# webmproject/sjpeg

Hardware: AMD Instinct MI355X
Metric: Mpixels/s JPEG encode, 4K RGB q=75 YUV420; bit-exact vs ref (higher is better)
Workload: dtype int32/int16 (u8 in); 1 GPU; 64 device-resident 3840x2160 G_struct frames per GPU per step, q=75 YUV420 method 0 (standard Huffman), one complete JPEG per frame; frames_per_gpu=64, width=3840, height=2160, yuv_mode=420, parallelism=frame-sharded x1, no data-path collective, pipelined=True

## Files before the change

sjpeg_amd/csrc/stitch_kernels.h:

```cpp

struct StitchArgs {
  int nseg, nframes;
  const uint32_t* seg_nbits;
  unsigned long long* seg_off;
  const uint32_t* seg_words;
  uint32_t slot_words;
  const uint32_t* pool;
  uint32_t pool_words;
  const uint32_t* seg_xbase;
  const uint32_t* pool_ctr;
  uint32_t* ubuf;
  size_t ubuf_words;
  uint32_t* chunk_ff;
  unsigned long long* chunk_off;
  uint32_t max_chunks;
  const uint8_t* header;
  uint32_t header_size;
  const uint32_t* hdr_off;
  int append_eoi;
  uint8_t* out;
  size_t out_stride;
  unsigned long long* sizes;
  unsigned long long* pack_off = nullptr;
  const unsigned long long* seg_nbits64;
  unsigned long long* total_bits_out;
  uint32_t subs;
  uint32_t wide_subs;
  int seg_first;
  int rst_tail;
  uint32_t* frame_flags;
  int fused_k4;
  int fused_k2;
  const RaggedFrame* rframes = nullptr;
  const uint32_t* rmap_place = nullptr;
  const uint32_t* rmap_stuff = nullptr;
};

__device__ __forceinline__ StitchArgs ragged_stitch_view(const StitchArgs& in, uint32_t f) {
  const RaggedFrame& d = in.rframes[f];
  StitchArgs v = in;
  v.nseg = d.nseg; v.nframes = 1;
  v.seg_nbits = in.seg_nbits + d.seg_base;
  v.seg_off = in.seg_off + d.seg_base + f;
  v.seg_words = in.seg_words + static_cast<size_t>(d.seg_base) * in.slot_words;
  v.pool = in.pool + d.pool_base; v.pool_words = d.pool_words;
  v.seg_xbase = in.seg_xbase + d.seg_base;
  v.pool_ctr = in.pool_ctr + 2 * f;
  v.ubuf = in.ubuf + d.ubuf_base; v.ubuf_words = d.ubuf_words;
  v.chunk_ff = in.chunk_ff + d.chunk_base; v.chunk_off = in.chunk_off + d.chunk_base; v.max_chunks = d.max_chunks;
  if (in.hdr_off != nullptr) v.hdr_off = in.hdr_off + f;
  v.out = in.out + d.out_offset; v.out_stride = d.out_capacity;
  v.sizes = in.sizes + f;
  v.frame_flags = in.frame_flags + f;
  return v;
}
__device__ __forceinline__ bool frame_overran(const StitchArgs& a, int frame) {
  if (a.pool_ctr == nullptr) return false;
  return a.frame_flags != nullptr ? a.frame_flags[frame] != 0u : a.pool_ctr[2 * frame + 1] != 0u;
}

template <bool RAGGED = false>
__global__ __launch_bounds__(kThreads) void scan_seg_offsets(const StitchArgs a_in) {
  __shared__ uint32_t scratch[16];
  const StitchArgs a = RAGGED ? ragged_stitch_view(a_in, blockIdx.x) : a_in;
  const int frame = RAGGED ? 0 : blockIdx.x;
  const uint32_t* nb = a.seg_nbits + static_cast<size_t>(frame) * a.nseg;
  unsigned long long* off = a.seg_off + static_cast<size_t>(frame) * (a.nseg + 1);
  auto len_of = [&](int i) -> uint32_t {
    return a.seg_nbits64 != nullptr ? static_cast<uint32_t>(a.seg_nbits64[static_cast<size_t>(frame) * a.nseg + i]) : nb[i];
  };
  constexpr int kRun = 8;
  unsigned long long running = 0;
  for (int base = 0; base < a.nseg; base += kThreads * kRun) {
    const int i0 = base + static_cast<int>(threadIdx.x) * kRun;
    uint32_t v[kRun];
    unsigned long long mine = 0;
#pragma unroll
    for (int j = 0; j < kRun; ++j) {
      v[j] = (i0 + j < a.nseg) ? len_of(i0 + j) : 0u;
      mine += v[j];
    }
    unsigned long long at, round_total;
    if (a.seg_nbits64 == nullptr) {
      uint32_t total;
      const uint32_t ex = wg_exclusive_scan<kThreads>(static_cast<uint32_t>(mine), scratch, &total);
      at = running + ex;
      round_total = total;
    } else {
      uint32_t total_lo, total_hi;
      const uint32_t ex_lo = wg_exclusive_scan<kThreads>(static_cast<uint32_t>(mine & 0xffffffu), scratch, &total_lo);
      const uint32_t ex_hi = wg_exclusive_scan<kThreads>(static_cast<uint32_t>(mine >> 24), scratch, &total_hi);
      at = running + ex_lo + (static_cast<unsigned long long>(ex_hi) << 24);
      round_total = total_lo + (static_cast<unsigned long long>(total_hi) << 24);
    }
#pragma unroll
    for (int j = 0; j < kRun; ++j) {
      if (i0 + j < a.nseg) off[i0 + j] = at;
      at += v[j];
    }
    running += round_total;
  }
  if (threadIdx.x == 0) {
    off[a.nseg] = running;
    if (a.total_bits_out != nullptr) a.total_bits_out[frame] = running;
  }
  const unsigned long long U = (running + 7) >> 3;
  unsigned long long nch64 = (U + kChunkBytes - 1) / kChunkBytes;
  if (nch64 > a.max_chunks) nch64 = a.max_chunks;
  const uint32_t nchunks = static_cast<uint32_t>(nch64);
  uint32_t* ff = a.chunk_ff + static_cast<size_t>(frame) * a.max_chunks;
  for (uint32_t i = threadIdx.x; i < nchunks; i += kThreads) ff[i] = 0;
  if (a.frame_flags != nullptr && a.pool_ctr != nullptr && threadIdx.x == 0) {
    a.frame_flags[frame] = a.pool_ctr[2 * frame + 1];
    const_cast<uint32_t*>(a.pool_ctr)[2 * frame] = 0u;
    const_cast<uint32_t*>(a.pool_ctr)[2 * frame + 1] = 0u;
  }
}


__device__ __forceinline__ uint32_t ff_bytes(uint32_t w) {
  return ((w & 0x7f7f7f7fu) + 0x01010101u) & w & 0x80808080u;
}
__device__ __forceinline__ uint32_t count_ff(uint32_t w, int nbytes ) {
  uint32_t n = 0;
#pragma unroll
  for (int b = 0; b < 4; ++b) {
    if (b < nbytes && ((w >> (24 - 8 * b)) & 0xffu) == 0xffu) ++n;
  }
  return n;
}

constexpr int kSpec = 12;
constexpr int kPlaceLanes = 64;
constexpr int kWideSpec = 3;
struct __attribute__((packed, aligned(4))) Words4 { uint32_t w[4]; };
constexpr int kFusedSegs = 2048;
constexpr int kFusedSegsBig = 16384;
template <int FUSED, bool RAGGED = false>
__global__ __launch_bounds__(kThreads) void place_segments(const StitchArgs a_in) {
  __shared__ uint32_t off_lds[FUSED == 1 ? kFusedSegs + 1 : 16];
  __shared__ uint32_t scratch_k2[16];
  const uint32_t rf = RAGGED ? a_in.rmap_place[blockIdx.x] : 0u;
  const uint32_t bx = RAGGED ? blockIdx.x - a_in.rframes[rf].place_base : blockIdx.x;
  const StitchArgs a = RAGGED ? ragged_stitch_view(a_in, rf) : a_in;
  const int frame = RAGGED ? 0 : blockIdx.y;
  const uint32_t* const nb_f = a.seg_nbits + static_cast<size_t>(frame) * a.nseg;
  const int sc_first = static_cast<int>((bx * (kThreads / 64)) / a.subs);
  if (FUSED == 1) {
    const uint32_t* const nb = nb_f;
    constexpr int kRun = kFusedSegs / kThreads;
    const int i0 = static_cast<int>(threadIdx.x) * kRun;
    uint32_t v[kRun], mine = 0;
#pragma unroll
    for (int j = 0; j < kRun; ++j) {
      v[j] = (i0 + j < a.nseg) ? nb[i0 + j] : 0u;
      mine += v[j];
    }
    uint32_t total;
    uint32_t at = wg_exclusive_scan<kThreads>(mine, scratch_k2, &total);
#pragma unroll
    for (int j = 0; j < kRun; ++j) { off_lds[i0 + j] = at; at += v[j]; }
    if (threadIdx.x == 0) {
      off_lds[a.nseg] = total;
      if (bx == 0) {
        a.seg_off[static_cast<size_t>(frame) * (a.nseg + 1) + a.nseg] = total;
        if (a.frame_flags != nullptr && a.pool_ctr != nullptr) a.frame_flags[frame] = a.pool_ctr[2 * frame + 1];
      }
    }
    __syncthreads();
  }
  if (FUSED == 2) {
    uint32_t front = 0, all = 0;
    for (int i = threadIdx.x; i < a.nseg; i += kThreads) {
      const uint32_t v = nb_f[i];
      all += v;
      front += i < sc_first ? v : 0u;
    }
    uint32_t front_total, all_total;
    (void)wg_exclusive_scan<kThreads>(front, scratch_k2, &front_total);
    (void)wg_exclusive_scan<kThreads>(all, scratch_k2, &all_total);
    if (threadIdx.x < 8) {
      uint32_t at = front_total;
      for (int j = 0; j < static_cast<int>(threadIdx.x); ++j) at += sc_first + j < a.nseg ? nb_f[sc_first + j] : 0u;
      off_lds[threadIdx.x] = at;
    }
    if (threadIdx.x == 8) {
      off_lds[8] = all_total;
      if (bx == 0) {
        a.seg_off[static_cast<size_t>(frame) * (a.nseg + 1) + a.nseg] = all_total;
        if (a.frame_flags != nullptr && a.pool_ctr != nullptr) a.frame_flags[frame] = a.pool_ctr[2 * frame + 1];
      }
    }
    __syncthreads();
  }
  const uint32_t unit = bx * (kThreads / kPlaceLanes) + (threadIdx.x >> 6);
  const int sc0 = static_cast<int>(unit / a.subs);
  const uint32_t ibase = (unit % a.subs) * (a.wide_subs ? kWideSpec * 256u : kSpec * kPlaceLanes);
  if (sc0 >= a.nseg) return;
  const unsigned long long* const off_g = a.seg_off + static_cast<size_t>(frame) * (a.nseg + 1);
  auto off = [&](int i) -> unsigned long long {
    if (FUSED == 1) return off_lds[i];
    if (FUSED == 2) {
      if (i >= a.nseg) return off_lds[8];
      if (i - sc_first < 8) return off_lds[i - sc_first];
      unsigned long long at = off_lds[7];
      for (int j = sc_first + 7; j < i; ++j) at += nb_f[j];
      return at;
    }
    return off_g[i];
  };
  const uint32_t* segw = a.seg_words + static_cast<size_t>(frame) * a.nseg * a.slot_words;
  const uint32_t* src = segw + static_cast<size_t>(sc0) * a.slot_words;
  const bool wide = (a.subs == 1u || a.wide_subs) && (a.slot_words & 3u) == 0u && a.slot_words >= 776u;
  uint32_t spec[kSpec][2];
  uint4 wq[kWideSpec];
  uint32_t wx[kWideSpec];
  if (wide) {
#pragma unroll
    for (int k = 0; k < kWideSpec; ++k) {
      const uint32_t i = min(ibase + 256u * k + 4u * (threadIdx.x & 63), a.slot_words - 4u);
      wq[k] = *reinterpret_cast<const uint4*>(src + i);
      wx[k] = src[min(i + 4u, a.slot_words - 1u)];
    }
  } else {
#pragma unroll
    for (int k = 0; k < kSpec; ++k) {
      const uint32_t i = min(ibase + k * kPlaceLanes + (threadIdx.x & 63), a.slot_words - 2u);
      spec[k][0] = src[i];
      spec[k][1] = src[i + 1];
    }
  }
  const bool has_next = sc0 + 1 < a.nseg;
  const uint32_t next_first = has_next ? src[a.slot_words] : 0u;
  const unsigned long long b0 = off(sc0), b1 = off(sc0 + 1);
  const unsigned long long b2 = off(has_next ? sc0 + 2 : sc0 + 1);
  const unsigned long long T = off(a.nseg);
  const unsigned long long U = (T + 7) >> 3;
  const bool overran = FUSED ? (a.pool_ctr != nullptr && a.pool_ctr[2 * frame + 1] != 0u) : frame_overran(a, frame);
  if (((U + 3) >> 2) + 1 > a.ubuf_words || overran) return;
  const uint32_t* const pool_f = a.pool == nullptr ? nullptr : a.pool + static_cast<size_t>(frame) * a.pool_words;
  const uint32_t* const xbase_f = a.seg_xbase == nullptr ? nullptr : a.seg_xbase + static_cast<size_t>(frame) * a.nseg;
  auto seg_word = [&](int sc, uint32_t i) -> uint32_t {
    if (i < a.slot_words) return segw[static_cast<size_t>(sc) * a.slot_words + i];
    if (xbase_f == nullptr) return 0u;
    const uint32_t xb = xbase_f[sc];
    return xb == 0xffffffffu ? 0u : pool_f[xb + (i - a.slot_words)];
  };
  uint32_t* ub = a.ubuf + static_cast<size_t>(frame) * a.ubuf_words;
  uint32_t* cff = a.chunk_ff + static_cast<size_t>(frame) * a.max_chunks;
  const int lane = threadIdx.x & 63;
  const unsigned long long wbeg = (b0 + 31) >> 5;
  const unsigned long long wend = (sc0 == a.nseg - 1) ? ((U + 3) >> 2) : ((b1 + 31) >> 5);
  const uint32_t nwords = static_cast<uint32_t>(wend - wbeg);
  const uint32_t lead = static_cast<uint32_t>(wbeg * 32 - b0);
  const uint32_t len = static_cast<uint32_t>(b1 - b0);
  uint32_t* dst = ub + wbeg;
  const uint32_t wbase = static_cast<uint32_t>(wbeg);
  uint32_t ff_acc = 0;
  uint32_t ff_chunk = 0xffffffffu;
  auto ff_flush = [&]() {
    uint32_t sum = ff_acc;
    for (int d = 32; d > 0; d >>= 1) sum += __shfl_down(sum, d, 64);
    if (lane == 0 && sum != 0u) atomicAdd(&cff[ff_chunk], sum);
    ff_acc = 0;
  };
  auto gather_word = [&](uint32_t i) -> uint32_t {
    uint32_t outw = 0;
    int need = 32, sc = sc0;
    unsigned long long p = (wbeg + i) * 32, c_beg = b0, c_end = b1;
    while (need > 0 && p < T) {
      while (p >= c_end) { ++sc; c_beg = c_end; c_end = off(sc + 1); }
      const unsigned long long avail = c_end - p;
      const int take = avail < static_cast<unsigned long long>(need) ? static_cast<int>(avail) : need;
      const uint32_t rr = static_cast<uint32_t>(p - c_beg);
      const unsigned long long two = (static_cast<unsigned long long>(seg_word(sc, rr >> 5)) << 32) | seg_word(sc, (rr >> 5) + 1);
      const uint32_t bits = static_cast<uint32_t>((two << (rr & 31)) >> (64 - take));
      outw |= bits << (need - take);
      need -= take;
      p += take;
    }
    if (need > 0) outw |= (need == 32) ? 0xffffffffu : ((1u << need) - 1u);
    return outw;
  };
  auto one = [&](uint32_t i, uint32_t v0, uint32_t v1) {
    uint32_t ffs = 0;
    if (i < nwords) {
      const uint32_t r = lead + 32u * i;
      uint32_t outw;
      if (r + 32u <= len) {
        outw = lead ? __builtin_amdgcn_alignbit(v0, v1, 32u - lead) : v0;
      } else {
        outw = gather_word(i);
      }
      dst[i] = outw;
      const unsigned long long byte0 = (wbeg + i) * 4;
      const int valid = byte0 >= U ? 0 : (U - byte0 >= 4 ? 4 : static_cast<int>(U - byte0));
      ffs = valid == 4 ? static_cast<uint32_t>(__popc(ff_bytes(outw))) : count_ff(outw, valid);
    }
    const uint32_t chunk = (wbase + i) >> 10;
    const uint32_t chunk0 = __builtin_amdgcn_readfirstlane(chunk);
    if (chunk0 != ff_chunk) {
      if (ff_chunk != 0xffffffffu) ff_flush();
      ff_chunk = chunk0;
    }
    if (chunk == chunk0) ff_acc += ffs;
    else if (ffs != 0u) atomicAdd(&cff[chunk], ffs);
  };
  const bool long_seg = ((len + lead + 31u) >> 5) + 2u > a.slot_words;
  if (!long_seg && wide) {
    const uint32_t n_int = len >= lead + 32u ? (len - lead) >> 5 : 0u;
    const uint32_t edge_bits = len > lead ? (len - lead) & 31u : 0u;
    const bool edge_easy = !has_next || (b2 - b1) >= 32u - edge_bits;
    const unsigned long long edge_byte0 = (wbeg + n_int) * 4;
    const uint32_t edge_valid = edge_byte0 >= U ? 0u : (U - edge_byte0 >= 4 ? 4u : static_cast<uint32_t>(U - edge_byte0));
    auto batch = [&](uint32_t i0, uint4 q, uint32_t x) {
      const uint32_t i = i0 + 4u * lane;
      const uint32_t v[5] = {q.x, q.y, q.z, q.w, x};
      const bool full = i0 + 256u <= n_int;
      Words4 o;
      uint32_t f[4];
#pragma unroll
      for (int u = 0; u < 4; ++u) {
        o.w[u] = lead ? __builtin_amdgcn_alignbit(v[u], v[u + 1], 32u - lead) : v[u];
        f[u] = static_cast<uint32_t>(__popc(ff_bytes(o.w[u])));
      }
      if (full) {
        *reinterpret_cast<Words4*>(dst + i) = o;
      } else {
        const bool edge_here = n_int < nwords && n_int >= i0 && n_int < i0 + 256u;
        const uint32_t gathered = (edge_here && !edge_easy) ? gather_word(n_int) : 0u;
        const uint32_t hi_mask = edge_bits ? ~(0xffffffffu >> edge_bits) : 0u;
        const uint32_t tail = (has_next ? next_first : 0xffffffffu) >> edge_bits;
#pragma unroll
        for (int u = 0; u < 4; ++u) {
          const uint32_t idx = i + u;
          if (edge_here && idx == n_int) {
            o.w[u] = edge_easy ? ((o.w[u] & hi_mask) | tail) : gathered;
            f[u] = edge_valid == 4u ? static_cast<uint32_t>(__popc(ff_bytes(o.w[u]))) : count_ff(o.w[u], static_cast<int>(edge_valid));
          }
          if (idx < nwords) dst[idx] = o.w[u]; else f[u] = 0;
        }
      }
      const uint32_t ffs = f[0] + f[1] + f[2] + f[3];
      const uint32_t c_lo = (wbase + i) >> 10, c_hi = (wbase + i + 3u) >> 10;
      const uint32_t chunk0 = __builtin_amdgcn_readfirstlane(c_lo);
      if (chunk0 != ff_chunk) {
        if (ff_chunk != 0xffffffffu) ff_flush();
        ff_chunk = chunk0;
      }
      if (c_lo == chunk0 && c_hi == chunk0) {
        ff_acc += ffs;
      } else if (ffs != 0u) {
#pragma unroll
        for (int u = 0; u < 4; ++u) {
          const uint32_t c = (wbase + i + u) >> 10;
          if (f[u] != 0u) { if (c == chunk0) ff_acc += f[u]; else atomicAdd(&cff[c], f[u]); }
        }
      }
    };
#pragma unroll
    for (int k = 0; k < kWideSpec; ++k) {
      if (ibase + 256u * k < nwords) batch(ibase + 256u * k, wq[k], wx[k]);
    }
    if (a.wide_subs) { if (ff_chunk != 0xffffffffu) ff_flush(); return; }
    auto fetch = [&](uint32_t i0, uint4* q, uint32_t* x) {
      const uint32_t i = min(i0 + 4u * lane, a.slot_words - 4u);
      *q = *reinterpret_cast<const uint4*>(src + i);
      *x = src[min(i + 4u, a.slot_words - 1u)];
    };
    uint4 qn = make_uint4(0, 0, 0, 0);
    uint32_t xn = 0;
    if (256u * kWideSpec < nwords) fetch(256u * kWideSpec, &qn, &xn);
    for (uint32_t i0 = 256u * kWideSpec; i0 < nwords; i0 += 256u) {
      const uint4 qc = qn;
      const uint32_t xc = xn;
      if (i0 + 256u < nwords) fetch(i0 + 256u, &qn, &xn);
      batch(i0, qc, xc);
    }
  } else if (!long_seg) {
#pragma unroll
    for (int k = 0; k < kSpec; ++k) {
      if (ibase + static_cast<uint32_t>(k) * kPlaceLanes < nwords) one(ibase + k * kPlaceLanes + lane, spec[k][0], spec[k][1]);
    }
    if (a.subs == 1u) {
      for (uint32_t i0 = kSpec * kPlaceLanes; i0 < nwords; i0 += kPlaceLanes) {
        const uint32_t i = i0 + lane;
        one(i, src[i], src[i + 1]);
      }
    }
  } else {
    const bool takes_rest = a.subs == 1u || (a.wide_subs && (unit % a.subs) == a.subs - 1u);
    const uint32_t iend = takes_rest ? nwords : min(nwords, ibase + kSpec * kPlaceLanes);
    for (uint32_t i0 = ibase; i0 < iend; i0 += kPlaceLanes) {
      const uint32_t i = i0 + lane;
      one(i, seg_word(sc0, i), seg_word(sc0, i + 1));
    }
  }
  if (ff_chunk != 0xffffffffu) ff_flush();
}

__device__ __forceinline__ uint8_t* frame_out(const StitchArgs& a, int frame) {
  return a.pack_off != nullptr ? a.out + a.pack_off[frame] : a.out + static_cast<size_t>(frame) * a.out_stride;
}


template <bool RAGGED = false>
__global__ __launch_bounds__(kThreads) void scan_chunk_offsets(const StitchArgs a_in) {
  __shared__ uint32_t scratch[16];
  const StitchArgs a = RAGGED ? ragged_stitch_view(a_in, blockIdx.x) : a_in;
  const int frame = RAGGED ? 0 : blockIdx.x;
  const unsigned long long T = a.seg_off[static_cast<size_t>(frame) * (a.nseg + 1) + a.nseg];
  const unsigned long long U = (T + 7) >> 3;
  unsigned long long nch64 = (U + kChunkBytes - 1) / kChunkBytes;
  if (nch64 > a.max_chunks) nch64 = a.max_chunks;
  const uint32_t nchunks = static_cast<uint32_t>(nch64);
  const uint32_t* ff = a.chunk_ff + static_cast<size_t>(frame) * a.max_chunks;
  unsigned long long* co = a.chunk_off + static_cast<size_t>(frame) * a.max_chunks;
  constexpr uint32_t kRun = 8;
  unsigned long long running = 0;
  for (uint32_t base = 0; base < nchunks; base += kThreads * kRun) {
    const uint32_t i0 = base + threadIdx.x * kRun;
    uint32_t v[kRun], mine = 0;
#pragma unroll
    for (uint32_t j = 0; j < kRun; ++j) {
      v[j] = (i0 + j < nchunks) ? ff[i0 + j] : 0u;
      mine += v[j];
    }
    uint32_t total;
    const uint32_t ex = wg_exclusive_scan<kThreads>(mine, scratch, &total);
    unsigned long long at = running + ex;
#pragma unroll
    for (uint32_t j = 0; j < kRun; ++j) {
      if (i0 + j < nchunks) co[i0 + j] = at;
      at += v[j];
    }
    running += total;
  }
  const unsigned long long body = U + running;
  const uint32_t hoff = a.hdr_off ? a.hdr_off[frame] : 0u;
  const uint32_t hsize = a.hdr_off ? a.hdr_off[frame + 1] - hoff : a.header_size;
  const unsigned long long size = hsize + body + (a.append_eoi ? 2 : 0);
  const bool fits = size <= a.out_stride && ((U + 3) >> 2) + 1 <= a.ubuf_words && !frame_overran(a, frame);
  __syncthreads();
  if (a.frame_flags == nullptr && a.pool_ctr != nullptr && threadIdx.x == 0) {
    const_cast<uint32_t*>(a.pool_ctr)[2 * frame] = 0u;
    const_cast<uint32_t*>(a.pool_ctr)[2 * frame + 1] = 0u;
  }
  if (threadIdx.x == 0) a.sizes[frame] = fits ? size : 0ull;
  if (a.pack_off != nullptr) return;
  uint8_t* dst = a.out + static_cast<size_t>(frame) * a.out_stride;
  if (threadIdx.x == 0 && fits && a.append_eoi) {
    dst[hsize + body] = 0xff;
    dst[hsize + body + 1] = 0xd9;
  }
  if (fits) {
    for (uint32_t i = threadIdx.x; i < hsize; i += kThreads) dst[i] = a.header[hoff + i];
  }
}

__global__ __launch_bounds__(kThreads) void pack_frame_offsets(const StitchArgs a) {
  __shared__ uint32_t scratch[16];
  unsigned long long running = 0;
  for (int f0 = 0; f0 < a.nframes; f0 += kThreads) {
    const int f = f0 + static_cast<int>(threadIdx.x);
    const unsigned long long mine = f < a.nframes ? ((a.sizes[f] + 15ull) & ~15ull) : 0ull;
    uint32_t total;
    const uint32_t ex = wg_exclusive_scan<kThreads>(static_cast<uint32_t>(mine >> 4), scratch, &total);
    if (f < a.nframes) a.pack_off[f] = running + (static_cast<unsigned long long>(ex) << 4);
    running += static_cast<unsigned long long>(total) << 4;
  }
  if (threadIdx.x == 0) a.pack_off[a.nframes] = running;
}

__global__ __launch_bounds__(kThreads) void pack_frame_edges(const StitchArgs a) {
  const int frame = blockIdx.x;
  const unsigned long long size = a.sizes[frame];
  if (size == 0) return;
  const uint32_t hoff = a.hdr_off ? a.hdr_off[frame] : 0u;
  const uint32_t hsize = a.hdr_off ? a.hdr_off[frame + 1] - hoff : a.header_size;
  uint8_t* const dst = a.out + a.pack_off[frame];
  for (uint32_t i = threadIdx.x; i < hsize; i += kThreads) dst[i] = a.header[hoff + i];
  if (threadIdx.x == 0 && a.append_eoi) { dst[size - 2] = 0xff; dst[size - 1] = 0xd9; }
  const uint32_t pad = static_cast<uint32_t>((16u - (size & 15u)) & 15u);
  if (threadIdx.x < pad) dst[size + threadIdx.x] = 0;
}


constexpr uint32_t kFusedChunks = 2048;
constexpr uint32_t kFusedChunksBig = 1u << 17;
template <int FUSED, bool RAGGED = false>
__global__ __launch_bounds__(kThreads) void stuff_chunks(const StitchArgs a_in) {
  constexpr uint32_t kCapChunks = FUSED == 2 ? kFusedChunksBig : kFusedChunks;
  __shared__ uint32_t scratch[16];
  __shared__ __attribute__((aligned(16))) uint8_t stage[2 * kChunkBytes + 64];
  __shared__ uint32_t fused_off[FUSED == 1 ? kFusedChunks : 1];
  uint32_t big_off = 0;
  const uint32_t rf = RAGGED ? a_in.rmap_stuff[blockIdx.x] : 0u;
  const uint32_t bx = RAGGED ? blockIdx.x - a_in.rframes[rf].stuff_base : blockIdx.x;
  const StitchArgs a = RAGGED ? ragged_stitch_view(a_in, rf) : a_in;
  const int frame = RAGGED ? 0 : blockIdx.y;
  const unsigned long long T = a.seg_off[static_cast<size_t>(frame) * (a.nseg + 1) + a.nseg];
  const unsigned long long U = (T + 7) >> 3;
  const uint32_t nchunks = static_cast<uint32_t>((U + kChunkBytes - 1) / kChunkBytes);
  const uint32_t* ub = a.ubuf + static_cast<size_t>(frame) * a.ubuf_words;
  const unsigned long long* co = a.chunk_off + static_cast<size_t>(frame) * a.max_chunks;
  const uint32_t hoff = a.hdr_off ? a.hdr_off[frame] : 0u;
  const uint32_t hsize = a.hdr_off ? a.hdr_off[frame + 1] - hoff : a.header_size;
  const uint32_t* const ff_f = a.chunk_ff + static_cast<size_t>(frame) * a.max_chunks;
  if (FUSED) {
    const uint32_t* ff = ff_f;
    const uint32_t nch = nchunks < a.max_chunks ? nchunks : a.max_chunks;
    uint32_t total;
    if (FUSED == 1) {
      constexpr uint32_t kRun = kFusedChunks / kThreads;
      const uint32_t i0 = threadIdx.x * kRun;
      uint32_t v[kRun], mine = 0;
#pragma unroll
      for (uint32_t j = 0; j < kRun; ++j) {
        v[j] = (i0 + j < nch) ? ff[i0 + j] : 0u;
        mine += v[j];
      }
      uint32_t at = wg_exclusive_scan<kThreads>(mine, scratch, &total);
#pragma unroll
      for (uint32_t j = 0; j < kRun; ++j) { fused_off[i0 + j] = at; at += v[j]; }
    } else {
      uint32_t front = 0, all = 0;
      for (uint32_t i = threadIdx.x; i < nch; i += kThreads) {
        const uint32_t v = ff[i];
        all += v;
        front += i < bx ? v : 0u;
      }
      (void)wg_exclusive_scan<kThreads>(front, scratch, &big_off);
      (void)wg_exclusive_scan<kThreads>(all, scratch, &total);
    }
    const unsigned long long body = U + total;
    const unsigned long long size = hsize + body + (a.append_eoi ? 2 : 0);
    const bool fits = nchunks <= kCapChunks && size <= a.out_stride && ((U + 3) >> 2) + 1 <= a.ubuf_words && !frame_overran(a, frame);
    if (bx == 0) {
      if (threadIdx.x == 0) a.sizes[frame] = fits ? size : 0ull;
      if (a.fused_k2 && a.pool_ctr != nullptr && threadIdx.x == 0) {
        const_cast<uint32_t*>(a.pool_ctr)[2 * frame] = 0u;
        const_cast<uint32_t*>(a.pool_ctr)[2 * frame + 1] = 0u;
      }
      if (fits) {
        uint8_t* const dst = a.out + static_cast<size_t>(frame) * a.out_stride;
        if (threadIdx.x == 0 && a.append_eoi) { dst[hsize + body] = 0xff; dst[hsize + body + 1] = 0xd9; }
        for (uint32_t i = threadIdx.x; i < hsize; i += kThreads) dst[i] = a.header[hoff + i];
      }
    }
    if (!fits) return;
    __syncthreads();
  } else {
    if (a.sizes[frame] == 0) return;
  }
  uint8_t* const dst0 = frame_out(a, frame) + hsize;
  auto fetch = [&](uint32_t chunk, uint4* q, uint32_t* behind, int* valid, unsigned long long* off) {
    *q = make_uint4(0, 0, 0, 0);
    *behind = 0;
    *valid = 0;
    *off = 0;
    if (chunk >= nchunks) return;
    const unsigned long long w0 = static_cast<unsigned long long>(chunk) * kChunkWords + threadIdx.x * 4;
    const unsigned long long byte0 = w0 * 4;
    *off = FUSED == 1 ? static_cast<unsigned long long>(fused_off[chunk]) : FUSED == 2 ? 0ull : co[chunk];
    if (byte0 < U) {
      *q = *reinterpret_cast<const uint4*>(ub + w0);
      *valid = (U - byte0 >= 16) ? 16 : static_cast<int>(U - byte0);
      if (byte0 + 16 < U) *behind = ub[w0 + 4];
    }
  };
  uint4 q_next;
  uint32_t behind_next;
  int valid_next;
  unsigned long long off_next;
  auto gdx_of = [&]() -> uint32_t { return RAGGED ? a_in.rframes[rf].stuff_wgs : gridDim.x; };
  fetch(bx, &q_next, &behind_next, &valid_next, &off_next);
  for (uint32_t chunk = bx; chunk < nchunks; chunk += gdx_of()) {
    const uint4 q = q_next;
    const uint32_t behind = behind_next;
    const int valid = valid_next;
    const unsigned long long chunk_off = FUSED == 2 ? static_cast<unsigned long long>(big_off) : off_next;
    fetch(chunk + gdx_of(), &q_next, &behind_next, &valid_next, &off_next);
    if (FUSED == 2 && chunk + gdx_of() < nchunks) {
      uint32_t mine = 0, step;
      for (uint32_t i = chunk + threadIdx.x; i < chunk + gdx_of(); i += kThreads) mine += ff_f[i];
      (void)wg_exclusive_scan<kThreads>(mine, scratch, &step);
      big_off += step;
    }
    const uint32_t w[4] = {q.x, q.y, q.z, q.w};
    uint32_t ffs = 0;
    if (valid == 16) {
#pragma unroll
      for (int j = 0; j < 4; ++j) ffs += __popc(ff_bytes(w[j]));
    } else {
#pragma unroll
      for (int j = 0; j < 4; ++j) ffs += count_ff(w[j], valid - 4 * j);
    }
    uint32_t total_ff;
    const uint32_t ex = wg_exclusive_scan<kThreads>(ffs, scratch, &total_ff);
    uint8_t* const dchunk = dst0 + static_cast<unsigned long long>(chunk) * kChunkBytes + chunk_off;
    const uint32_t mis = static_cast<uint32_t>(reinterpret_cast<uintptr_t>(dchunk) & 15u);
    const uint32_t o = mis + threadIdx.x * 16 + ex;
    const uint32_t n0 = behind >> 24, n1 = (behind >> 16) & 0xffu, n2 = (behind >> 8) & 0xffu;
    const bool behind_plain = (ff_bytes(behind) & 0x80808000u) == 0u;
    if (valid == 16 && ffs == 0u && behind_plain) {
      const uint32_t m[5] = {__builtin_bswap32(w[0]), __builtin_bswap32(w[1]), __builtin_bswap32(w[2]),
                             __builtin_bswap32(w[3]), __builtin_bswap32(behind)};
      const uint32_t up = (0u - o) & 3u;
      uint32_t d[4];
#pragma unroll
      for (int k = 0; k < 4; ++k) d[k] = __builtin_amdgcn_alignbyte(m[k + 1], m[k], up);
      uint32_t* const sp = reinterpret_cast<uint32_t*>(stage + o + up);
      sp[0] = d[0]; sp[1] = d[1]; sp[2] = d[2]; sp[3] = d[3];
      if (threadIdx.x == 0) {
        for (uint32_t j = 0; j < up; ++j) stage[o + j] = static_cast<uint8_t>(m[0] >> (8 * j));
      }
    } else {
      uint8_t* sp = stage + o;
#pragma unroll
      for (int j = 0; j < 16; ++j) {
        if (j < valid) {
          const uint8_t b = static_cast<uint8_t>(w[j >> 2] >> (24 - 8 * (j & 3)));
          *sp++ = b;
          if (b == 0xff) *sp++ = 0x00;
        }
      }
      sp[0] = static_cast<uint8_t>(n0);
      sp[1] = static_cast<uint8_t>(n0 == 0xffu ? 0u : n1);
      sp[2] = static_cast<uint8_t>(n0 == 0xffu ? n1 : (n1 == 0xffu ? 0u : n2));
    }
    __syncthreads();
    const unsigned long long rest = U - static_cast<unsigned long long>(chunk) * kChunkBytes;
    const uint32_t nbytes = static_cast<uint32_t>(rest < kChunkBytes ? rest : kChunkBytes) + total_ff;
    uint8_t* const dalign = dchunk - mis;
    const uint32_t lo = mis, hi = mis + nbytes;
    const uint32_t first_full = (lo + 15u) & ~15u, last_full = hi & ~15u;
    if (first_full <= last_full) {
      for (uint32_t i = first_full / 16 + threadIdx.x; i < last_full / 16; i += kThreads) {
        reinterpret_cast<uint4*>(dalign)[i] = reinterpret_cast<const uint4*>(stage)[i];
      }
      if (threadIdx.x < first_full - lo) dalign[lo + threadIdx.x] = stage[lo + threadIdx.x];
      if (threadIdx.x < hi - last_full) dalign[last_full + threadIdx.x] = stage[last_full + threadIdx.x];
    } else {
      if (threadIdx.x < nbytes) dalign[lo + threadIdx.x] = stage[lo + threadIdx.x];
    }
    __syncthreads();
  }
}



__global__ __launch_bounds__(kThreads) void patch_restart_markers(const StitchArgs a) {
  const int frame = blockIdx.y;
  const int s = static_cast<int>(blockIdx.x * (kThreads / 64) + (threadIdx.x >> 6));
  const int lane = threadIdx.x & 63;
  if (s >= a.nseg - (a.rst_tail ? 0 : 1) || a.sizes[frame] == 0) return;
  const unsigned long long end_bits = a.seg_off[static_cast<size_t>(frame) * (a.nseg + 1) + s + 1];
  const unsigned long long p = (end_bits >> 3) - 2;
  const unsigned long long chunk = p / kChunkBytes, cstart = chunk * kChunkBytes;
  const uint32_t* ub = a.ubuf + static_cast<size_t>(frame) * a.ubuf_words;
  uint32_t ffs = 0;
  for (unsigned long long b = cstart + 4ull * lane; b < p; b += 256) {
    const unsigned long long left = p - b;
    ffs += count_ff(ub[b >> 2], left >= 4 ? 4 : static_cast<int>(left));
  }
  for (int d = 32; d > 0; d >>= 1) ffs += __shfl_down(ffs, d, 64);
  if (lane == 0) {
    const uint32_t hsize = a.hdr_off ? a.hdr_off[frame + 1] - a.hdr_off[frame] : a.header_size;
    uint8_t* dst = frame_out(a, frame) + hsize + p +
                   a.chunk_off[static_cast<size_t>(frame) * a.max_chunks + chunk] + ffs;
    dst[0] = 0xff;
    dst[1] = static_cast<uint8_t>(0xd0 + ((s + a.seg_first) & 7));
  }
}
```

Before: 598,400 Mpixels/s.

## Rewrite unfused byte-stuffing as wave-per-chunk kernel with register permutes

For the non-fused path, stuff_chunks now assigns each wavefront whole chunks, walked in 1 KiB steps with 16 bytes per lane. Lanes find 0xFF bytes with bit tricks, compute their output shift with ballot and mbcnt prefix counts, and insert zero bytes using byte permutes in registers. Stores go straight to global memory, without the LDS staging buffer and block-wide syncs of the old path. Loads are prefetched two steps ahead, and the kernel gains an amdgpu_waves_per_eu(8) occupancy hint. The cost is much more complex alignment and tail-handling logic, with some risk of register pressure.

```diff
diff --git a/sjpeg_amd/csrc/stitch_kernels.h b/sjpeg_amd/csrc/stitch_kernels.h
--- a/sjpeg_amd/csrc/stitch_kernels.h
+++ b/sjpeg_amd/csrc/stitch_kernels.h
@@ -489,7 +489,7 @@
 constexpr uint32_t kFusedChunks = 2048;
 constexpr uint32_t kFusedChunksBig = 1u << 17;
 template <int FUSED, bool RAGGED = false>
-__global__ __launch_bounds__(kThreads) void stuff_chunks(const StitchArgs a_in) {
+__device__ __forceinline__ void stuff_fused(const StitchArgs& a_in) {
   constexpr uint32_t kCapChunks = FUSED == 2 ? kFusedChunksBig : kFusedChunks;
   __shared__ uint32_t scratch[16];
   __shared__ __attribute__((aligned(16))) uint8_t stage[2 * kChunkBytes + 64];
@@ -648,6 +648,145 @@
   }
 }
 
+constexpr uint32_t kStuffStep = 1024;
+
+template <int N>
+__device__ __forceinline__ void stuff_lane(const uint32_t (&m)[5], uint32_t M, uint32_t up, uint32_t L, bool head,
+                                           uint8_t* const A, const uint8_t* const dend) {
+  uint32_t D[N + 1];
+  D[0] = __builtin_amdgcn_alignbyte(m[0], 0u, up);
+#pragma unroll
+  for (int t = 0; t < N; ++t) D[t + 1] = __builtin_amdgcn_alignbyte(t + 1 < 5 ? m[t + 1] : 0u, t < 5 ? m[t] : 0u, up);
+  for (int it = 0; __ballot(M != 0u) != 0ull; ++it) {
+    const int r = M != 0u ? __ffs(M) + it - static_cast<int>(up) : (1 << 20);
+    M &= M - 1u;
+    const int ts = r >> 2;
+    const uint32_t rr = static_cast<uint32_t>(r) & 3u;
+    const uint32_t keep = static_cast<uint32_t>(0x01010101ull >> (32u - 8u * rr));
+    const uint32_t sel = ((0x06050403u + keep) & ~(0xffu << (8u * rr))) | (0x0cu << (8u * rr));
+#pragma unroll
+    for (int t = N - 1; t >= -1; --t) {
+      D[t + 1] = __builtin_amdgcn_perm(D[t + 1], t >= 0 ? D[t] : 0u, t < ts ? 0x07060504u : (t == ts ? sel : 0x06050403u));
+    }
+  }
+  if (head) {
+    for (uint32_t b = 0; b < up; ++b) {
+      if (A + b < dend) A[b] = static_cast<uint8_t>(D[0] >> (8 * (4 - up + b)));
+    }
+  }
+  const uint32_t n = L > up ? (L - up + 3u) >> 2 : 0u;
+  uint8_t* const p = A + up;
+  const bool whole4 = n >= 4u && p + 16 <= dend;
+  if (whole4) {
+    Words4 o;
+    o.w[0] = D[1]; o.w[1] = D[2]; o.w[2] = D[3]; o.w[3] = D[4];
+    *reinterpret_cast<Words4*>(p) = o;
+  }
+#pragma unroll
+  for (int t = 0; t < N; ++t) {
+    if (static_cast<uint32_t>(t) < n && !(whole4 && t < 4)) {
+      uint8_t* const q = p + 4 * t;
+      if (q + 4 <= dend) {
+        *reinterpret_cast<uint32_t*>(q) = D[t + 1];
+      } else {
+        for (int b = 0; b < 3; ++b) {
+          if (q + b < dend) q[b] = static_cast<uint8_t>(D[t + 1] >> (8 * b));
+        }
+      }
+    }
+  }
+}
+
+template <bool RAGGED>
+__device__ __forceinline__ void stuff_waves(const StitchArgs& a_in) {
+  const uint32_t rf = RAGGED ? a_in.rmap_stuff[blockIdx.x] : 0u;
+  const uint32_t bx = RAGGED ? blockIdx.x - a_in.rframes[rf].stuff_base : blockIdx.x;
+  const StitchArgs a = RAGGED ? ragged_stitch_view(a_in, rf) : a_in;
+  const int frame = RAGGED ? 0 : blockIdx.y;
+  const unsigned long long size = a.sizes[frame];
+  if (size == 0) return;
+  const unsigned long long T = a.seg_off[static_cast<size_t>(frame) * (a.nseg + 1) + a.nseg];
+  const unsigned long long U = (T + 7) >> 3;
+  const uint32_t nchunks = static_cast<uint32_t>((U + kChunkBytes - 1) / kChunkBytes);
+  const uint32_t* const ub = a.ubuf + static_cast<size_t>(frame) * a.ubuf_words;
+  const unsigned long long* const co = a.chunk_off + static_cast<size_t>(frame) * a.max_chunks;
+  const uint32_t hsize = a.hdr_off ? a.hdr_off[frame + 1] - a.hdr_off[frame] : a.header_size;
+  uint8_t* const dst0 = frame_out(a, frame) + hsize;
+  const uint8_t* const dend = frame_out(a, frame) + size - (a.append_eoi ? 2 : 0);
+  const uint32_t lane = threadIdx.x & 63;
+  constexpr uint32_t kWaves = kThreads / 64;
+  const uint32_t wstride = (RAGGED ? a_in.rframes[rf].stuff_wgs : gridDim.x) * kWaves;
+  const uint32_t c0 = bx * kWaves + (threadIdx.x >> 6);
+  if (c0 >= nchunks) return;
+  const uint32_t nk = 4 * ((nchunks - c0 + wstride - 1) / wstride);
+  auto fetch = [&](uint32_t k, uint4* q, uint32_t* behind) {
+    *q = make_uint4(0, 0, 0, 0);
+    *behind = 0;
+    const uint32_t c = c0 + (k >> 2) * wstride;
+    const unsigned long long byte0 = static_cast<unsigned long long>(c) * kChunkBytes + (k & 3u) * kStuffStep + 16u * lane;
+    if (k < nk && byte0 < U) {
+      *q = *reinterpret_cast<const uint4*>(ub + (byte0 >> 2));
+      if (byte0 + 16 < U) *behind = ub[(byte0 >> 2) + 4];
+    }
+  };
+  uint4 qa, qb;
+  uint32_t ha, hb;
+  fetch(0, &qa, &ha);
+  fetch(1, &qb, &hb);
+  unsigned long long coff_ahead = co[c0];
+  unsigned long long dpos = 0;
+  for (uint32_t k = 0; k < nk; ++k) {
+    const uint4 cq = qa;
+    const uint32_t cb = ha;
+    qa = qb;
+    ha = hb;
+    fetch(k + 2, &qb, &hb);
+    const uint32_t chunk = c0 + (k >> 2) * wstride, s = k & 3u;
+    if (s == 0) {
+      dpos = static_cast<unsigned long long>(chunk) * kChunkBytes + coff_ahead;
+      coff_ahead = chunk + wstride < nchunks ? co[chunk + wstride] : 0ull;
+    }
+    const unsigned long long sbyte0 = static_cast<unsigned long long>(chunk) * kChunkBytes + s * kStuffStep;
+    if (sbyte0 >= U) break;
+    const unsigned long long byte0 = sbyte0 + 16u * lane;
+    const uint32_t valid = byte0 >= U ? 0u : (U - byte0 >= 16 ? 16u : static_cast<uint32_t>(U - byte0));
+    const uint32_t m[5] = {__builtin_bswap32(cq.x), __builtin_bswap32(cq.y), __builtin_bswap32(cq.z),
+                           __builtin_bswap32(cq.w), __builtin_bswap32(cb)};
+    const uint32_t g01 = ((ff_bytes(m[1]) | (ff_bytes(m[0]) >> 4)) * 0x204081u) >> 24;
+    const uint32_t g23 = ((ff_bytes(m[3]) | (ff_bytes(m[2]) >> 4)) * 0x204081u) >> 24;
+    const uint32_t g4 = ((ff_bytes(m[4]) & 0x8080u) * 0x204u) & 0x30000u;
+    const uint32_t M = (g01 | (g23 << 8) | g4) & (valid >= 16u ? 0x3ffffu : (1u << valid) - 1u);
+    const uint32_t c = static_cast<uint32_t>(__popc(M & 0xffffu));
+    uint32_t ex, tot;
+    const unsigned long long b0 = __ballot((c & 1u) != 0u);
+    if (__ballot(c > 1u) == 0ull) {
+      ex = __builtin_amdgcn_mbcnt_hi(static_cast<uint32_t>(b0 >> 32), __builtin_amdgcn_mbcnt_lo(static_cast<uint32_t>(b0), 0u));
+      tot = static_cast<uint32_t>(__popcll(b0));
+    } else {
+      ex = 0;
+      tot = 0;
+#pragma unroll
+      for (int bit = 4; bit >= 0; --bit) {
+        const unsigned long long bb = __ballot(((c >> bit) & 1u) != 0u);
+        ex = __builtin_amdgcn_mbcnt_hi(static_cast<uint32_t>(bb >> 32), __builtin_amdgcn_mbcnt_lo(static_cast<uint32_t>(bb), 2u * ex));
+        tot = 2u * tot + static_cast<uint32_t>(__popcll(bb));
+      }
+    }
+    uint8_t* const A = dst0 + dpos + 16u * lane + ex;
+    const uint32_t up = (0u - static_cast<uint32_t>(reinterpret_cast<uintptr_t>(A))) & 3u;
+    const bool head = sbyte0 == 0 && lane == 0;
+    if (__ballot(c > 4u) == 0ull) stuff_lane<5>(m, M, up, valid + c, head, A, dend);
+    else stuff_lane<8>(m, M, up, valid + c, head, A, dend);
+    dpos += kStuffStep + tot;
+  }
+}
+
+template <int FUSED, bool RAGGED = false>
+__global__ __launch_bounds__(kThreads) __attribute__((amdgpu_waves_per_eu(8))) void stuff_chunks(const StitchArgs a_in) {
+  if constexpr (FUSED == 0) stuff_waves<RAGGED>(a_in);
+  else stuff_fused<FUSED, RAGGED>(a_in);
+}
+
 
 
 __global__ __launch_bounds__(kThreads) void patch_restart_markers(const StitchArgs a) {
```

Result: faster. 605,700 Mpixels/s, median of 6 (+1.2%).
